# Distributed-Deep-Learning/ps

Measured on AMD Instinct MI355X. Metric: samples/sec (whole node) ResNet-50 sync-BSP at 1/2/4/8 MI355X workers, higher is better.
Workload: dtype bf16; 1 GPU; model=ResNet-50, global_batch=1024, image_size=224, parallelism=ps-bsp-colocated-dp1, optimizer=momentum@lr:0.1@momentum:0.9@wd:5e-05@nesterov:0.0@, staleness=0, fused_bn=True, ranks_per_device=1, compute_priority=high, side_stream=True, streams_per_rank=3, data_plane=local

## Files before the change

### csrc/kernels/conv_bwd_fused.hip

```cpp
#include <algorithm>
#include <cstdlib>

#include "psamd_device.h"
#include "psamd_launch.h"

namespace psamd {
namespace {

typedef float f32x16 __attribute__((ext_vector_type(16)));
typedef short s16x4 __attribute__((ext_vector_type(4)));
typedef short s16x8 __attribute__((ext_vector_type(8)));
typedef short s16x8i __attribute__((ext_vector_type(8)));
typedef __attribute__((address_space(1))) const void gptr_t;
typedef __attribute__((address_space(3))) void lptr_t;
typedef __attribute__((address_space(3))) const char lds_char;

__device__ __attribute__((aligned(16))) uint16_t kZeroRow[8] = {0, 0, 0, 0, 0, 0, 0, 0};

constexpr int kTM = 128;
constexpr int kKS = 64;
constexpr int kNW = 8;
constexpr int kSlot = kTM * kKS * 2;

__device__ __forceinline__ int swf(int r) {
  const int y = (r >> 1) & 7;
  return y ^ ((y & 1) << 2);
}

__device__ __forceinline__ uint32_t lds_addr(const void* p) {
  return static_cast<uint32_t>(reinterpret_cast<uintptr_t>((lds_char*)p));
}

__device__ __forceinline__ bf16x8_t ld_b128(uint32_t a) {
  bf16x8_t v;
  asm volatile("ds_read_b128 %0, %1" : "=v"(v) : "v"(a) : "memory");
  return v;
}
__device__ __forceinline__ f32x4 ld_f4(uint32_t a) {
  f32x4 v;
  asm volatile("ds_read_b128 %0, %1" : "=v"(v) : "v"(a) : "memory");
  return v;
}
__device__ __forceinline__ s16x4 ld_b64(uint32_t a) {
  s16x4 v;
  asm volatile("ds_read_b64 %0, %1" : "=v"(v) : "v"(a) : "memory");
  return v;
}
__device__ __forceinline__ s16x4 ld_tr(uint32_t a) {
  s16x4 v;
  asm volatile("ds_read_b64_tr_b16 %0, %1" : "=v"(v) : "v"(a) : "memory");
  return v;
}
__device__ __forceinline__ void st_b128(uint32_t a, bf16x8_t v) {
  asm volatile("ds_write_b128 %0, %1" ::"v"(a), "v"(v) : "memory");
}
__device__ __forceinline__ void lgkm0() { asm volatile("s_waitcnt lgkmcnt(0)" ::: "memory"); }
template <typename T>
__device__ __forceinline__ void tie(T& v) {
  asm volatile("" : "+v"(v));
}
template <int N>
__device__ __forceinline__ void wait_vm() {
  asm volatile("s_waitcnt vmcnt(%0)" ::"n"(N) : "memory");
}
__device__ __forceinline__ void lds_bar() {
  asm volatile("s_waitcnt lgkmcnt(0)" ::: "memory");
  __builtin_amdgcn_s_barrier();
  asm volatile("" ::: "memory");
}

__device__ __forceinline__ bf16x8_t cat8(s16x4 lo, s16x4 hi) {
  return __builtin_bit_cast(bf16x8_t, s16x8{lo[0], lo[1], lo[2], lo[3], hi[0], hi[1], hi[2], hi[3]});
}

template <int CI, int CO, bool PLAIN>
__global__ __launch_bounds__(512, 1) void conv11_bwd_fused_kernel(const Conv11BwdArgs p) {
  static_assert(CI == 64 && CO == 256, "the layer-1 conv3 shape (64 -> 256): 4 stages per tile");
  constexpr int NS = CO / kKS;
  constexpr int NR = 5, PD = NR - 1;
  constexpr int WROW = CO * 2;
  constexpr int W_BYTES = CI * WROW;
  constexpr int RING = W_BYTES;
  constexpr int Z2 = RING + NR * kSlot;
  constexpr int PAR = Z2 + 2 * kSlot;
  constexpr int NPAR = 3 * CO + 4 * CI;
  constexpr int LDS_BYTES = PAR + NPAR * 4;
  static_assert(LDS_BYTES <= 163840, "LDS budget");
  static_assert(4 * NS * 16 * 64 * 4 <= (NR + 2) * kSlot, "dW half-sum scratch fits the ring + z2 slots");
  __shared__ __attribute__((aligned(16))) uint8_t lds[LDS_BYTES];
  float* const par = reinterpret_cast<float*>(lds + PAR);
  const uint32_t L0 = lds_addr(lds);

  const int t = threadIdx.x, lane = t & 63, wave = __builtin_amdgcn_readfirstlane(t >> 6);
  const int fr = lane & 31, fh = lane >> 5;
  const int GM = gridDim.x, mg = blockIdx.x;
  const int ntiles = (p.M + kTM - 1) / kTM;
  const int my_tiles = mg < ntiles ? (ntiles - mg + GM - 1) / GM : 0;
  const int nq = my_tiles * NS;
  auto stage_m0 = [&](int q) { return q < nq ? (mg + (q / NS) * GM) * kTM : p.M; };

  for (int i = t; i < NPAR; i += kNW * 64) {
    float v;
    if (i < 3 * CO) v = p.cbwd[i];
    else if (PLAIN) v = 0.f;
    else if (i < 3 * CO + 2 * CI) v = p.cf2[i - 3 * CO];
    else if (i < 3 * CO + 3 * CI) v = p.mean2[i - 3 * CO - 2 * CI];
    else v = p.invstd2[i - 3 * CO - 3 * CI];
    par[i] = v;
  }
  {
    constexpr int CPR = CO / 8, RPP = 64 / CPR, PPW = W_BYTES / 1024 / kNW;
    const int lr = lane / CPR, lp = lane % CPR;
#pragma unroll
    for (int i = 0; i < PPW; ++i) {
      const int k = wave * PPW + i, r = k * RPP + lr;
      __builtin_amdgcn_global_load_lds((gptr_t*)(p.wt + static_cast<int64_t>(r) * CO + (lp ^ (r & 15)) * 8),
                                       (lptr_t*)(lds + k * 1024), 16, 0, 0);
    }
  }
  auto issue_tile = [&](const uint16_t* base, int stride, int col0, int m0, int dst) {
#pragma unroll
    for (int i = 0; i < 2; ++i) {
      const int k = wave * 2 + i, r = 8 * k + (lane >> 3), m = m0 + r;
      const int lc = (lane & 7) ^ swf(r);
      const uint16_t* src = m < p.M ? base + static_cast<int64_t>(m) * stride + col0 + lc * 8 : kZeroRow;
      __builtin_amdgcn_global_load_lds((gptr_t*)src, (lptr_t*)(lds + dst + k * 1024), 16, 0, 0);
    }
  };
  const int zr = t >> 3, zc = t & 7;
  u16x8 z3r[2][2];
  auto load_z3 = [&](int q, u16x8 (&dst)[2]) {
    const int m0 = stage_m0(q), col = (q % NS) * kKS + zc * 8;
#pragma unroll
    for (int i = 0; i < 2; ++i) {
      const int m = m0 + zr + 64 * i;
      dst[i] = m < p.M ? *reinterpret_cast<const u16x8*>(p.z3 + static_cast<int64_t>(m) * CO + col)
                       : u16x8{0, 0, 0, 0, 0, 0, 0, 0};
    }
  };
  issue_tile(p.z2, CI, 0, stage_m0(0), Z2);
#pragma unroll
  for (int i = 0; i < PD; ++i) issue_tile(p.g, CO, (i % NS) * kKS, stage_m0(i), RING + i * kSlot);
  load_z3(0, z3r[0]);
  load_z3(1, z3r[1]);
  wait_vm<0>();
  lds_bar();

  const int pb = wave & 3, cbd = wave >> 2;
  const int nb = wave & 1, cw = (wave >> 1) & 1, khw = wave >> 2;
  const int dpx = 32 * pb + fr, dsw = swf(dpx);
  const uint32_t wrow = L0 + static_cast<uint32_t>((32 * cbd + fr) * WROW);
  const int gi = lane >> 4, i16 = lane & 15;
  const int trow = 8 * (gi >> 1) + (i16 >> 2), tcol = 16 * (gi & 1) + 4 * (i16 & 3);
  auto tr_off = [&](int c0, int h) {
    const int r = trow + 4 * h;
    return static_cast<uint32_t>(r * 128 + ((((c0 + tcol) >> 3) ^ swf(r)) << 4) + (tcol & 7) * 2);
  };
  const uint32_t tD0 = tr_off(32 * nb, 0), tD1 = tr_off(32 * nb, 1);
  const uint32_t tZ0 = tr_off(32 * cw, 0), tZ1 = tr_off(32 * cw, 1);
  const float asc = par[3 * CO + 32 * cw + fr], ash = par[3 * CO + CI + 32 * cw + fr];

  f32x16 acc_dg, accW[NS];
  auto zero16 = [](f32x16& a) {
#pragma unroll
    for (int i = 0; i < 16; ++i) a[i] = 0.f;
  };
  zero16(acc_dg);
#pragma unroll
  for (int s = 0; s < NS; ++s) zero16(accW[s]);
  const int ec = 32 * cbd + fr;
  const float emc = par[3 * CO + ec], esh = par[3 * CO + CI + ec], emu = par[3 * CO + 2 * CI + ec],
              eis = par[3 * CO + 3 * CI + ec];
  float s1 = 0.f, s2 = 0.f;

  bf16x8_t a2f[4];
  auto make_a2 = [&](int ti) {
    const uint32_t zs = L0 + Z2 + (ti & 1) * kSlot + khw * (4 * 2048);
    s16x4 lo[4], hi[4];
#pragma unroll
    for (int ks = 0; ks < 4; ++ks) {
      lo[ks] = ld_tr(zs + ks * 2048 + tZ0);
      hi[ks] = ld_tr(zs + ks * 2048 + tZ1);
    }
    lgkm0();
#pragma unroll
    for (int ks = 0; ks < 4; ++ks) {
      tie(lo[ks]);
      tie(hi[ks]);
      if constexpr (PLAIN) {
        a2f[ks] = cat8(lo[ks], hi[ks]);
        continue;
      }
      u16x8 v = __builtin_bit_cast(u16x8, cat8(lo[ks], hi[ks]));
#pragma unroll
      for (int j = 0; j < 8; ++j) v[j] = f32_to_bf16(bf16_to_f32(v[j]) * asc + ash);
      const s16x8i z = {0, 0, 0, 0, 0, 0, 0, 0};
      a2f[ks] = __builtin_bit_cast(bf16x8_t, __builtin_elementwise_max(__builtin_bit_cast(s16x8i, v), z));
    }
  };
  auto transform = [&](int sl, int s, int m0, const u16x8 (&z3v)[2]) {
    const uint32_t ds = L0 + RING + sl * kSlot;
    const uint32_t pa = L0 + PAR + (s * kKS + zc * 8) * 4;
    const f32x4 ca0 = ld_f4(pa), ca1 = ld_f4(pa + 16);
    const f32x4 cb0 = ld_f4(pa + CO * 4), cb1 = ld_f4(pa + CO * 4 + 16);
    const f32x4 cc0 = ld_f4(pa + 2 * CO * 4), cc1 = ld_f4(pa + 2 * CO * 4 + 16);
    bf16x8_t gv[2];
    uint32_t ga[2];
#pragma unroll
    for (int i = 0; i < 2; ++i) {
      const int r = zr + 64 * i;
      ga[i] = ds + r * 128 + ((zc ^ swf(r)) << 4);
      gv[i] = ld_b128(ga[i]);
    }
    lgkm0();
    f32x4 c0a = ca0, c0b = ca1, c1a = cb0, c1b = cb1, c2a = cc0, c2b = cc1;
    tie(c0a); tie(c0b); tie(c1a); tie(c1b); tie(c2a); tie(c2b);
#pragma unroll
    for (int i = 0; i < 2; ++i) {
      tie(gv[i]);
      const u16x8 g8 = __builtin_bit_cast(u16x8, gv[i]);
      const u16x8 z8 = z3v[i];
      u16x8 d;
#pragma unroll
      for (int j = 0; j < 8; ++j) {
        const float a = j < 4 ? c0a[j] : c0b[j - 4], b = j < 4 ? c1a[j] : c1b[j - 4], c = j < 4 ? c2a[j] : c2b[j - 4];
        d[j] = f32_to_bf16(a * bf16_to_f32(g8[j]) + b * bf16_to_f32(z8[j]) + c);
      }
      if (m0 + zr + 64 * i >= p.M) d = u16x8{0, 0, 0, 0, 0, 0, 0, 0};
      st_b128(ga[i], __builtin_bit_cast(bf16x8_t, d));
    }
  };
  auto compute = [&](int sl, f32x16& aw, int s) {
    const uint32_t ds = L0 + RING + sl * kSlot;
#pragma unroll
    for (int h = 0; h < 2; ++h) {
      bf16x8_t wa[2], xb[2];
      s16x4 dlo[2], dhi[2];
#pragma unroll
      for (int k2 = 0; k2 < 2; ++k2) {
        const int ks = 2 * h + k2;
        wa[k2] = ld_b128(wrow + ((((8 * s + 2 * ks + fh) ^ (fr & 15))) << 4));
        xb[k2] = ld_b128(ds + dpx * 128 + (((2 * ks + fh) ^ dsw) << 4));
        dlo[k2] = ld_tr(ds + (4 * khw + ks) * 2048 + tD0);
        dhi[k2] = ld_tr(ds + (4 * khw + ks) * 2048 + tD1);
      }
      lgkm0();
#pragma unroll
      for (int k2 = 0; k2 < 2; ++k2) {
        tie(wa[k2]);
        tie(xb[k2]);
        tie(dlo[k2]);
        tie(dhi[k2]);
      }
#pragma unroll
      for (int k2 = 0; k2 < 2; ++k2)
        acc_dg = __builtin_amdgcn_mfma_f32_32x32x16_bf16(xb[k2], wa[k2], acc_dg, 0, 0, 0);
#pragma unroll
      for (int k2 = 0; k2 < 2; ++k2)
        aw = __builtin_amdgcn_mfma_f32_32x32x16_bf16(cat8(dlo[k2], dhi[k2]), a2f[2 * h + k2], aw, 0, 0, 0);
    }
  };
  auto epilogue = [&](int ti) {
    const int m0 = (mg + ti * GM) * kTM;
    if constexpr (PLAIN) {
#pragma unroll
      for (int q = 0; q < 16; ++q) {
        const int m = m0 + 32 * pb + 8 * (q >> 2) + 4 * fh + (q & 3);
        if (m < p.M) p.gy[static_cast<int64_t>(m) * CI + ec] = f32_to_bf16(acc_dg[q]);
      }
      zero16(acc_dg);
      return;
    }
    const uint32_t zs = L0 + Z2 + (ti & 1) * kSlot;
    s16x4 zv[4];
#pragma unroll
    for (int q4 = 0; q4 < 4; ++q4) {
      const int r = 32 * pb + 8 * q4 + 4 * (gi >> 1) + (i16 >> 2);
      const int col = 32 * cbd + 16 * (gi & 1) + 4 * (i16 & 3);
      zv[q4] = ld_tr(zs + r * 128 + (((col >> 3) ^ swf(r)) << 4) + (col & 7) * 2);
    }
    lgkm0();
#pragma unroll
    for (int q4 = 0; q4 < 4; ++q4) {
      tie(zv[q4]);
      const u16x4 z4 = __builtin_bit_cast(u16x4, zv[q4]);
#pragma unroll
      for (int e = 0; e < 4; ++e) {
        const uint16_t val = f32_to_bf16(acc_dg[4 * q4 + e]);
        const float z = bf16_to_f32(z4[e]);
        const bool on = z * emc + esh > 0.f;
        const float gv = on ? bf16_to_f32(val) : 0.f;
        s1 += gv;
        s2 += gv * ((z - emu) * eis);
        const int m = m0 + 32 * pb + 8 * q4 + 4 * fh + e;
        if (m < p.M) p.gy[static_cast<int64_t>(m) * CI + ec] = on ? val : static_cast<uint16_t>(0);
      }
    }
    zero16(acc_dg);
  };

  int sl = 0, q = 0;
  for (int ti = 0; ti < my_tiles; ++ti) {
    const int m0 = (mg + ti * GM) * kTM;
#pragma unroll
    for (int s = 0; s < NS; ++s, ++q) {
      if (s == 0) make_a2(ti);
      transform(sl, s, m0, z3r[s & 1]);
      lds_bar();
      const int slp = sl == 0 ? NR - 1 : sl - 1;
      issue_tile(p.g, CO, ((q + PD) % NS) * kKS, stage_m0(q + PD), RING + slp * kSlot);
      load_z3(q + 2, z3r[s & 1]);
      if (s == 0) issue_tile(p.z2, CI, 0, ti + 1 < my_tiles ? m0 + GM * kTM : p.M, Z2 + ((ti + 1) & 1) * kSlot);
      compute(sl, accW[s], s);
      if (s == NS - 1) epilogue(ti);
      if (s == NS - 1) wait_vm<6>();
      else wait_vm<8>();
      lds_bar();
      sl = sl == NR - 1 ? 0 : sl + 1;
    }
  }
  wait_vm<0>();
  lds_bar();

  s1 += __shfl_xor(s1, 32, 64);
  s2 += __shfl_xor(s2, 32, 64);
  float* red = reinterpret_cast<float*>(lds + RING);
  if (!PLAIN && fh == 0) {
    red[pb * CI + ec] = s1;
    red[(4 + pb) * CI + ec] = s2;
  }
  __syncthreads();
  if (!PLAIN && t < CI) {
    p.part[static_cast<int64_t>(mg) * CI + t] = (red[t] + red[CI + t]) + (red[2 * CI + t] + red[3 * CI + t]);
    p.part[static_cast<int64_t>(GM + mg) * CI + t] =
        (red[4 * CI + t] + red[5 * CI + t]) + (red[6 * CI + t] + red[7 * CI + t]);
  }
  __syncthreads();
  float* wsc = reinterpret_cast<float*>(lds + RING);
  if (khw == 1) {
#pragma unroll
    for (int s = 0; s < NS; ++s)
#pragma unroll
      for (int i = 0; i < 16; ++i) wsc[(((wave - 4) * NS + s) * 16 + i) * 64 + lane] = accW[s][i];
  }
  __syncthreads();
  if (khw == 0) {
    float* slab = p.ws + static_cast<int64_t>(mg) * CO * CI;
#pragma unroll
    for (int s = 0; s < NS; ++s)
#pragma unroll
      for (int i = 0; i < 16; ++i) {
        const int n = s * kKS + 32 * nb + 8 * (i >> 2) + 4 * fh + (i & 3);
        slab[n * CI + 32 * cw + fr] = accW[s][i] + wsc[((wave * NS + s) * 16 + i) * 64 + lane];
      }
  }
}

template <bool BF16>
__global__ __launch_bounds__(256) void slab_sum_kernel(const float* __restrict__ in, int nslab, int per, int64_t E,
                                                       void* __restrict__ out) {
  const int64_t e = static_cast<int64_t>(blockIdx.x) * 256 + threadIdx.x;
  if (e >= E) return;
  const int b0 = blockIdx.y * per, b1 = min(nslab, b0 + per);
  float a0 = 0.f, a1 = 0.f, a2 = 0.f, a3 = 0.f;
  int b = b0;
  for (; b + 3 < b1; b += 4) {
    a0 += in[b * E + e];
    a1 += in[(b + 1) * E + e];
    a2 += in[(b + 2) * E + e];
    a3 += in[(b + 3) * E + e];
  }
  for (; b < b1; ++b) a0 += in[b * E + e];
  const float v = (a0 + a1) + (a2 + a3);
  if constexpr (BF16) static_cast<uint16_t*>(out)[blockIdx.y * E + e] = f32_to_bf16(v);
  else static_cast<float*>(out)[blockIdx.y * E + e] = v;
}

int slab_levels(int nslab) { return nslab > 16 ? (nslab + 15) / 16 : 0; }

}

bool conv11_bwd_fused_ok(int CI, int CO) { return CI == 64 && CO == 256; }

bool conv11_bwd_plain_ok(int CI, int CO) { return CI == 64 && CO == 256; }

bool conv11_bwd_built(int CI, int CO) { return CI == 64 && CO == 256; }

int conv11_bwd_blocks(int M, int CI, int CO) {
  (void)CI, (void)CO;
  const int ntiles = (M + kTM - 1) / kTM;
  return std::max(1, std::min(ntiles, 256));
}

int64_t conv11_bwd_ws(int M, int CI, int CO) {
  const int gm = conv11_bwd_blocks(M, CI, CO);
  return static_cast<int64_t>(gm + slab_levels(gm)) * CI * CO;
}

void launch_conv11_bwd_fused(const Conv11BwdArgs& a, int CI, int CO, hipStream_t s) {
  if (a.M <= 0) return;
  const int gm = conv11_bwd_blocks(a.M, CI, CO);
  if (CI == 64 && CO == 256 && a.cf2 == nullptr)
    hipLaunchKernelGGL((conv11_bwd_fused_kernel<64, 256, true>), dim3(gm), dim3(512), 0, s, a);
  else if (CI == 64 && CO == 256) hipLaunchKernelGGL((conv11_bwd_fused_kernel<64, 256, false>), dim3(gm), dim3(512), 0, s, a);
  else if (a.cf2 == nullptr) return;
  else return;
  const int64_t E = static_cast<int64_t>(CI) * CO;
  const unsigned eb = static_cast<unsigned>((E + 255) / 256);
  const int groups = slab_levels(gm);
  if (groups) {
    float* mid = a.ws + static_cast<int64_t>(gm) * E;
    hipLaunchKernelGGL(slab_sum_kernel<false>, dim3(eb, groups), dim3(256), 0, s, a.ws, gm, 16, E,
                       static_cast<void*>(mid));
    hipLaunchKernelGGL(slab_sum_kernel<true>, dim3(eb), dim3(256), 0, s, mid, groups, groups, E,
                       static_cast<void*>(a.dw));
  } else {
    hipLaunchKernelGGL(slab_sum_kernel<true>, dim3(eb), dim3(256), 0, s, a.ws, gm, gm, E, static_cast<void*>(a.dw));
  }
}

}
```

### csrc/kernels/convgemm.hip

```cpp
#include <algorithm>
#include <cstdlib>
#include <type_traits>

#include "psamd_device.h"
#include "psamd_launch.h"

namespace psamd {
namespace {

typedef float f32x16 __attribute__((ext_vector_type(16)));
typedef short s16x4 __attribute__((ext_vector_type(4)));
typedef short s16x8 __attribute__((ext_vector_type(8)));
typedef __attribute__((address_space(3))) s16x4 lds_s16x4;

constexpr int kBM = 128;
constexpr int kBK = 64;
constexpr int kWM = 64;

__device__ __forceinline__ bf16x8_t as_bf16x8(s16x8 v) { return __builtin_bit_cast(bf16x8_t, v); }

__device__ __forceinline__ void lds_barrier() {
  asm volatile("s_waitcnt lgkmcnt(0)" ::: "memory");
  __builtin_amdgcn_s_barrier();
  asm volatile("" ::: "memory");
// ... 1202 lines not shown
  for (int st = 0; st < pre; ++st) issue(st, st);
  if constexpr (PROL) {
    if (pre == 3) wait_vmcnt<2 * PER>();
    else if (pre == 2) wait_vmcnt<PER>();
    else wait_vmcnt<0>();
    lds_barrier();
    if (nst > 0) xform(0);
  }
  for (int st = 0; st < nst; ++st) {
    const int ahead = min(WS - 2, nst - 1 - st);
    if constexpr (PROL) {
      if (ahead >= 2) wait_vmcnt<PER>();
      else wait_vmcnt<0>();
    } else {
      if (ahead >= 2) wait_vmcnt<2 * PER>();
      else if (ahead == 1) wait_vmcnt<PER>();
      else wait_vmcnt<0>();
    }
    lds_barrier();
    if (st + WS - 1 < nst) issue(st + WS - 1, (st + WS - 1) % WS);
    if constexpr (PROL) {
      if (st + 1 < nst) xform((st + 1) % WS);
    }
    if constexpr (DB) {
      if (dbt) {
        const uint16_t* Gs = lds + (st % WS) * STAGE;
        const int cc = t % GCPR;
#pragma unroll
        for (int r = t / GCPR; r < kWP; r += DBR) {
          const u16x8 v = *reinterpret_cast<const u16x8*>(Gs + r * BNO + ((cc ^ tr_swz<BNO>(r)) << 3));
#pragma unroll
          for (int j = 0; j < 8; ++j) dbacc[j] += bf16_to_f32(v[j]);
        }
      }
    }
    mma(st % WS);
  }
  if constexpr (DB) {
    if (dbt) {
      lds_barrier();
      float* red = reinterpret_cast<float*>(lds);
#pragma unroll
      for (int j = 0; j < 8; ++j) red[t * 8 + j] = dbacc[j];
      lds_barrier();
      if (t < BNO) {
        const int cc = t >> 3, j = t & 7;
        float sum = 0.f;
        for (int k = 0; k < DBR; ++k) sum += red[(k * GCPR + cc) * 8 + j];
        p.dbws[static_cast<int64_t>(split) * p.N + n0 + t] = sum;
      }
    }
  }
  float* sl = p.ws + static_cast<int64_t>(split) * p.N * p.K;
  const int h = lane >> 5, kl = lane & 31;
#pragma unroll
  for (int i = 0; i < TN; ++i)
#pragma unroll
    for (int j = 0; j < TK; ++j)
#pragma unroll
      for (int q = 0; q < 16; ++q) {
        const int n = n0 + wn + 32 * i + (q & 3) + 8 * (q >> 2) + 4 * h;
        sl[static_cast<int64_t>(n) * p.K + k0 + wk + 32 * j + kl] = acc[i][j][q];
      }
}

constexpr int kPP = 112;

template <int OFF>
__device__ __forceinline__ s16x4 ds_tr_off(uint32_t a) {
  s16x4 v;
  asm volatile("ds_read_b64_tr_b16 %0, %1 offset:%2" : "=v"(v) : "v"(a), "i"(OFF) : "memory");
  return v;
}

template <int W, int S>
__global__ __launch_bounds__(768, 1) void conv_wgrad_patch_kernel(const ConvWgradArgs p, int stages_per_split) {
  constexpr int OW = W / S, R = kPP / OW, PR = S * (R - 1) + 3;
  constexpr int PW = S == 1 ? W + 2 : (W + 2) / 2;
  constexpr int KPS = S == 1 ? 3 : 2;
  static_assert(kPP % OW == 0 && OW % 4 == 0 && W % S == 0, "a stage is whole rows; 4-pixel groups stay in a row");
  constexpr int GPL = kPP * 64;
  constexpr int GB = 2 * GPL;
  constexpr int PPL = S * PR * PW * 64;
  constexpr int PB = ((2 * PPL + 1023) / 1024) * 1024;
  constexpr int GI = GB / 1024, PI = PB / 1024;
  constexpr int NI = GI + PI;
  constexpr int STB = GB + PB;
  constexpr int MAXW = (NI + 11) / 12;
  static_assert(GB % 1024 == 0 && MAXW <= 8 && (KPS == 2 || MAXW <= 4) && KPS * STB <= 160 * 1024, "stage shape");
  __shared__ __attribute__((aligned(16))) uint16_t lds[KPS * STB / 2];

  const ConvGeo& g = p.g;
  const int t = threadIdx.x, lane = t & 63, wave = __builtin_amdgcn_readfirstlane(t >> 6);
  const int nct = g.C / 64, tiles = (p.N / 64) * nct;
  const int L = xcd_remap(blockIdx.x, gridDim.x);
  const int split = L / tiles, tile = L - split * tiles;
  const int n0 = (tile / nct) * 64, c0 = (tile % nct) * 64;
  const int rows_per_img = g.OH / R, total = p.M / kPP;
  const int sb = split * stages_per_split;
  const int se = min(total, sb + stages_per_split);
  const int nst = se > sb ? se - sb : 0;

  const int myn = (NI - wave + 11) / 12;
  auto issue = [&](int st, int buf) {
    const int q = sb + st, img = q / rows_per_img, ih0 = (q - img * rows_per_img) * R * S - 1;
    uint8_t* base = reinterpret_cast<uint8_t*>(lds) + buf * STB;
    const uint16_t* gsrc = p.dz + static_cast<int64_t>(q) * kPP * p.N + n0;
    const uint16_t* xsrc = p.x + (static_cast<int64_t>(img) * g.H + ih0) * g.W * g.C + c0;
#pragma unroll
    for (int j = 0; j < MAXW; ++j) {
      if (j >= myn) break;
      const int i = wave + 12 * j;
      const uint16_t* src;
      if (i < GI) {
        const int ch = i * 64 + lane, pl = ch / (GPL / 16), r = ch - pl * (GPL / 16);
        src = gsrc + static_cast<int64_t>(r >> 2) * p.N + pl * 32 + (r & 3) * 8;
      } else {
        const int ch = (i - GI) * 64 + lane, pl = ch / (PPL / 16), r = ch - pl * (PPL / 16), slot = r >> 2;
        const int par = slot / (PR * PW), rem = slot - par * (PR * PW), pr = rem / PW;
        const int pc = S * (rem - pr * PW) + par, ih = ih0 + pr;
        const bool ok = pl < 2 && pc >= 1 && pc <= W && static_cast<unsigned>(ih) < static_cast<unsigned>(g.H);
        src = ok ? xsrc + (static_cast<int64_t>(pr) * W + (pc - 1)) * g.C + pl * 32 + (r & 3) * 8 : kZeroPage;
      }
      __builtin_amdgcn_global_load_lds((gptr_t*)src, (lptr_t*)(base + i * 1024), 16, 0, 0);
    }
  };

  const int kh = wave % 3, nh = (wave / 3) & 1, chf = wave / 6;
  const int gi = lane >> 4, i16 = lane & 15;
  const int mrow = 8 * (gi >> 1) + (i16 >> 2), colb = (16 * (gi & 1) + 4 * (i16 & 3)) * 2;
  const uint32_t ga = static_cast<uint32_t>(nh * GPL + mrow * 64 + colb);
  uint32_t xa[7][2];
#pragma unroll
  for (int s = 0; s < 7; ++s)
#pragma unroll
    for (int h = 0; h < 2; ++h) {
      const int m = 16 * s + 4 * h + mrow, oh = m / OW, ow = m - oh * OW;
      xa[s][h] = static_cast<uint32_t>(GB + chf * PPL + ((S * oh + kh) * PW + ow) * 64 + colb);
    }

  f32x16 acc[3];
#pragma unroll
  for (int k = 0; k < 3; ++k)
#pragma unroll
    for (int q = 0; q < 16; ++q) acc[k][q] = 0.f;
  auto mma = [&](int buf) {
    const uint32_t b0 = static_cast<uint32_t>(reinterpret_cast<uintptr_t>((const lds_s16x4*)lds)) + buf * STB;
    const uint32_t gb = b0 + ga;
    constexpr int K1 = S == 1 ? 64 : PR * PW * 64, K2 = S == 1 ? 128 : 64;
#define PSAMD_PATCH_STEP(Q)                                                                              \
  {                                                                                                      \
    s16x4 a0 = ds_tr_off<(16 * Q) * 64>(gb), a1 = ds_tr_off<(16 * Q + 4) * 64>(gb);                      \
    const uint32_t x0 = b0 + xa[Q][0], x1 = b0 + xa[Q][1];                                               \
    s16x4 p00 = ds_tr_off<0>(x0), p01 = ds_tr_off<0>(x1);                                                \
    s16x4 p10 = ds_tr_off<K1>(x0), p11 = ds_tr_off<K1>(x1);                                              \
    s16x4 p20 = ds_tr_off<K2>(x0), p21 = ds_tr_off<K2>(x1);                                              \
       \
       \
    asm volatile("s_waitcnt lgkmcnt(0)"                                                                  \
                 : "+v"(a0), "+v"(a1), "+v"(p00), "+v"(p01), "+v"(p10), "+v"(p11), "+v"(p20), "+v"(p21)  \
                 :                                                                                       \
                 : "memory");                                                                            \
    const bf16x8_t af = as_bf16x8(s16x8{a0[0], a0[1], a0[2], a0[3], a1[0], a1[1], a1[2], a1[3]});        \
    acc[0] = __builtin_amdgcn_mfma_f32_32x32x16_bf16(                                                    \
        af, as_bf16x8(s16x8{p00[0], p00[1], p00[2], p00[3], p01[0], p01[1], p01[2], p01[3]}), acc[0], 0, 0, 0); \
    acc[1] = __builtin_amdgcn_mfma_f32_32x32x16_bf16(                                                    \
        af, as_bf16x8(s16x8{p10[0], p10[1], p10[2], p10[3], p11[0], p11[1], p11[2], p11[3]}), acc[1], 0, 0, 0); \
    acc[2] = __builtin_amdgcn_mfma_f32_32x32x16_bf16(                                                    \
        af, as_bf16x8(s16x8{p20[0], p20[1], p20[2], p20[3], p21[0], p21[1], p21[2], p21[3]}), acc[2], 0, 0, 0); \
  }
    PSAMD_PATCH_STEP(0)
    PSAMD_PATCH_STEP(1)
    PSAMD_PATCH_STEP(2)
    PSAMD_PATCH_STEP(3)
    PSAMD_PATCH_STEP(4)
    PSAMD_PATCH_STEP(5)
    PSAMD_PATCH_STEP(6)
#undef PSAMD_PATCH_STEP
  };

  const int pre = nst < KPS - 1 ? nst : KPS - 1;
  for (int st = 0; st < pre; ++st) issue(st, st);
  for (int st = 0; st < nst; ++st) {
    if (KPS == 3 && st + 1 < nst) {
      if (myn == 4) asm volatile("s_waitcnt vmcnt(4)" ::: "memory");
      else if (myn == 3) asm volatile("s_waitcnt vmcnt(3)" ::: "memory");
      else if (myn == 2) asm volatile("s_waitcnt vmcnt(2)" ::: "memory");
      else asm volatile("s_waitcnt vmcnt(0)" ::: "memory");
    } else {
      asm volatile("s_waitcnt vmcnt(0)" ::: "memory");
    }
    lds_barrier();
    if (st + KPS - 1 < nst) issue(st + KPS - 1, (st + KPS - 1) % KPS);
    mma(st % KPS);
  }
  float* sl = p.ws + static_cast<int64_t>(split) * p.N * p.K;
  const int h = lane >> 5, cl = lane & 31;
#pragma unroll
  for (int kw = 0; kw < 3; ++kw)
#pragma unroll
    for (int q = 0; q < 16; ++q) {
      const int n = n0 + nh * 32 + (q & 3) + 8 * (q >> 2) + 4 * h;
      const int k = (kh * 3 + kw) * g.C + c0 + chf * 32 + cl;
      sl[static_cast<int64_t>(n) * p.K + k] = acc[kw][q];
    }
// ... 439 lines not shown
```

### ps_amd/knobs.py

```python
from __future__ import annotations

import os
from typing import Dict, FrozenSet

ENV = "PS_AMD_DISABLE"

ROUTES: Dict[str, str] = {
    "fused_block": "bottlenecks module by module (nn.Conv2d on MIOpen + BatchNormAct2d)",
    "conv3x3": "fused blocks' 3x3 convolutions on MIOpen instead of the implicit-GEMM kernels",
    "block_out": "block outputs applied by their own pass, not in the next conv1's prologue",
    "fold_bn3": "bn3's backward reduce as its own pass, not in the consumer's conv1 data-gradient epilogue",
    "fold_bn_ds": "the downsample BN's backward reduce as its own pass (epilogue 8 instead of 9)",
    "conv3_bwd_fused": "conv3's data + weight gradient as two GEMMs (dz3 through HBM)",
    "ds_bwd_fused": "the downsample's data + weight gradient as apply pass + two GEMMs",
    "weight_prep": "backward weight layouts built per block instead of in one launch per forward",
    "pool_bn_bwd": "stem max-pool backward and BN backward as separate passes",
    "stem_bwd_fused": "stem weight gradient reading a materialised dz",
    "splitk_wgrad": "linear weight gradients on hipBLASLt instead of the split-K kernel",
    "linear_fork": "linear weight gradients on the compute stream",
    "fused_relu": "Linear + ReLU as separate ops",
    "ps_linear": "PS-owned linear weight gradients through autograd's ordinary accumulation",
    "fused_attn": "short-sequence attention on SDPA",
    "flash_attn": "causal GQA attention on SDPA",
    "fused_xent": "cross-entropy on fp32 logits through F.cross_entropy",
    "bag_pool": "multi-hot bags pooled by gather_rows -> weight multiply -> segment_reduce_rows ([nnz, dim] in HBM)",
}

_cache: Dict[str, FrozenSet[str]] = {}


def _parse(raw: str) -> FrozenSet[str]:
    got = _cache.get(raw)
    if got is None:
        got = frozenset(s.strip() for s in raw.split(",") if s.strip())
        bad = sorted(got - set(ROUTES))
        if bad:
            raise ValueError(f"{ENV}: unknown route(s) {bad}; known: {sorted(ROUTES)}")
        _cache[raw] = got
    return got


def disabled(route: str) -> bool:
    if route not in ROUTES:
        raise KeyError(f"unknown route {route!r}")
    raw = os.environ.get(ENV)
    return bool(raw) and route in _parse(raw)


def enabled(route: str) -> bool:
    return not disabled(route)
```

### ps_amd/ops/convgemm.py

```python
from __future__ import annotations

import contextlib
import enum
import threading
import weakref
from typing import List

import torch
import torch.nn as nn
import torch.nn.functional as F

from .. import knobs
from . import side_stream as _side
from ._ext import native


def rows(x: torch.Tensor) -> torch.Tensor:
    n, c, h, w = x.shape
    if not x.is_contiguous(memory_format=torch.channels_last):
        x = x.contiguous(memory_format=torch.channels_last)
    return x.permute(0, 2, 3, 1).reshape(n * h * w, c)


def image(y2: torch.Tensor, n: int, h: int, w: int) -> torch.Tensor:
# ... 64 lines not shown
                parts.append((((ar2 * 3 + kh) * 3 + kw) * c1 + ar1).reshape(-1))
        idx = _PHASE_IDX[key] = torch.cat(parts).to(w.device)
    flat = w.permute(0, 2, 3, 1).reshape(-1)[idx]
    out, o = [], 0
    for nh, nw in ((1, 1), (1, 2), (2, 1), (2, 2)):
        k = nh * nw * c2
        out.append(flat[o:o + c1 * k].view(c1, k))
        o += c1 * k
    return out


DGRAD_S2_MIN_C = 128

WGRAD3X3_MIN_C = 256

TWOSRC_MAX_N = 128

PRO_FUSE_MAX_K = 256


def _conv3x3_enabled() -> bool:
    return knobs.enabled("conv3x3")


class _Link:

    __slots__ = ("out_ref", "z3", "bits", "mean", "invstd", "part", "dx_ptr", "dx_version", "dx_keep", "zd", "md",
                 "idd")

    def __init__(self, z3, bits, mean, invstd, zd=None, md=None, idd=None):
        self.out_ref = None
        self.z3, self.bits, self.mean, self.invstd = z3, bits, mean, invstd
        self.zd, self.md, self.idd = zd, md, idd
        self.part = None
        self.dx_ptr = self.dx_version = self.dx_keep = None


FOLD_STATS = {"used": 0, "ds": 0, "resp": 0}


class _Deferred:

    __slots__ = ("out_ref", "z3", "cf3", "res", "cfd", "out", "bits")

    def __init__(self, z3, cf3, res, cfd, out, bits):
        self.out_ref = None
        self.z3, self.cf3, self.res, self.cfd, self.out, self.bits = z3, cf3, res, cfd, out, bits

    def flush(self) -> None:
        y, b = native().bn_apply_coef(self.z3, self.cf3, self.res, self.cfd, 1, True)
        with torch.no_grad():
            self.out.copy_(y)
            self.bits.copy_(b)


def _resp_enabled() -> bool:
    return knobs.enabled("block_out")


def big_tile(m: int, n: int, k: int, src2: int = Src2.NONE, epi: int = Epi.STATS, pro: bool = False) -> bool:
    return tuple(native().conv_gemm_plan(m, n, k, [m, 1, m, 1, 1, 1, 0], pro, int(epi), int(src2))[:2]) == (256, 256)


def resp_consumer_ok(blk: nn.Module, m: int = 0) -> bool:
    c1 = blk.conv1
    if m > 0 and big_tile(m, c1.out_channels, c1.in_channels, src2=Src2.BLOCK_OUT):
        return True
    return c1.out_channels <= TWOSRC_MAX_N and (
        c1.in_channels >= 64 * native().kTwosrcGldsMinNk or c1.out_channels <= 64)


def flush_deferred() -> None:
    pend = getattr(_tls, "pend", None)
    _tls.pend = None
    if pend is not None and pend.out_ref is not None and pend.out_ref() is not None:
        pend.flush()


def _bwd_prologue_enabled(n: int) -> bool:
    return n <= TWOSRC_MAX_N


def _conv3_bwd_fused(ci: int, co: int) -> bool:
    return knobs.enabled("conv3_bwd_fused") and bool(native().conv11_bwd_fused_supported(ci, co))


def _ds_bwd_fused(ci: int, co: int, s: int) -> bool:
    return (s == 1 and knobs.enabled("ds_bwd_fused")
            and bool(native().conv11_bwd_fused_supported(ci, co, True)))


def _fold_enabled() -> bool:
    return knobs.enabled("fold_bn3")


def _fold_ds_enabled() -> bool:
    return knobs.enabled("fold_bn_ds")


def _conv1_dgrad_epi(downsample: bool, stride: int, fold: bool, producer_ds: bool) -> Epi:
    if downsample:
        if stride == 2:
            return Epi.FOLD_ADD_S2 if fold else Epi.ADD_S2
        return Epi.FOLD_ADD if fold else Epi.ADD
    if not fold:
        return Epi.ADD_MASKED
    return Epi.FOLD_ADD_MASKED_DS if producer_ds else Epi.FOLD_ADD_MASKED


class _BottleneckFn(torch.autograd.Function):
    @staticmethod
    def forward(ctx, x, w1, g1, b1, w2, g2, b2, w3, g3, b3, wd, gd, bd, blk, link_in, pend_in):
        nat = native()
        n, cin, h, w = x.shape
        s = blk.conv2.stride[0]
        oh, ow = (h - 1) // s + 1, (w - 1) // s + 1
        gi, go = geo(h, w), geo(oh, ow)
        x2 = rows(x)
        bn1, bn2, bn3 = blk.bn1, blk.bn2, blk.bn3
        k1 = bn1.running_mean
        if pend_in is not None:
            z1, p1 = nat.conv_gemm(pend_in.z3, _mat(w1), gi, pro=pend_in.cf3, epi=Epi.STATS, kshift=k1,
                                   a2=pend_in.res, pro2=pend_in.cfd, aout=x2, abits=pend_in.bits)
            FOLD_STATS["resp"] += 1
        else:
            z1, p1 = nat.conv_gemm(x2, _mat(w1), gi, epi=Epi.STATS, kshift=k1)
        m1, i1, cf1 = _finalize(p1, k1, n * h * w, bn1)
        y1 = nat.bn_apply_coef(z1, cf1, None, None, 1)[0]
        if _conv3x3_enabled():
            k2 = bn2.running_mean
            z2r, p2s = nat.conv_gemm(y1, _mat3(w2), geo(h, w, 3, s, 1), epi=Epi.STATS, kshift=k2)
            m2, i2, cf2 = _finalize(p2s, k2, n * oh * ow, bn2)
        else:
            z2r = rows(F.conv2d(image(y1, n, h, w), w2, None, s, 1))
            m2, i2, cf2 = nat.bn_stats(z2r, g2, b2, bn2.running_mean, bn2.running_var, True, _momentum(bn2),
                                       float(bn2.eps))
        k3 = bn3.running_mean
        if z2r.shape[1] <= PRO_FUSE_MAX_K:
            z3, p3 = nat.conv_gemm(z2r, _mat(w3), go, pro=cf2, epi=Epi.STATS, kshift=k3)
        else:
            z3, p3 = nat.conv_gemm(nat.bn_apply_coef(z2r, cf2, None, None, 1)[0], _mat(w3), go, epi=Epi.STATS,
                                   kshift=k3)
        m3, i3, cf3 = _finalize(p3, k3, n * oh * ow, bn3)
        cfd = None
        if wd is not None:
            bnd = blk.downsample[1]
            kd = bnd.running_mean
            zd, pd = nat.conv_gemm(x2, _mat(wd), geo(h, w, 1, s), epi=Epi.STATS, kshift=kd)
            md, idd, cfd = _finalize(pd, kd, n * oh * ow, bnd)
        else:
            zd = md = idd = None
        if (getattr(blk, "_defer_out", False) and getattr(_tls, "pending", None) is not None
                and _resp_enabled()):
            out = torch.empty_like(z3)
            obits = torch.empty(z3.numel() // 8, dtype=torch.uint8, device=z3.device)
            _tls.pend_new = _Deferred(z3, cf3, zd if wd is not None else x2, cfd, out, obits)
        else:
            out, obits = nat.bn_apply_coef(z3, cf3, zd if wd is not None else x2, cfd, 1, True)
        ctx.save_for_backward(x2, w1, w2, w3, wd, g1, g2, g3, gd, z1, y1, z2r, z3, obits, zd,
                              m1, i1, cf1, m2, i2, cf2, m3, i3, md, idd)
        ctx.dims = (n, h, w, s, oh, ow)
        ctx.prep = _prep_for(blk, w1, w2, w3)
        ctx.link_in = link_in
        ctx.link_out = (_Link(z3, obits, m3, i3, zd if _fold_ds_enabled() else None, md, idd)
                        if _fold_enabled() else None)
        return image(out, n, oh, ow)
# ... 263 lines not shown
```

Before: 16910 samples/s.

## Extend fused conv3 backward kernel to layer-2 128->512 shape via channel halves

Generalizes the fused 1x1 conv3 data+weight-gradient backward kernel to the layer-2 shape (128 in, 512 out). It splits the input channels into two 64-wide halves handled by paired blocks and uses a 3-slot ring to fit LDS. Per-lane constants are re-read from LDS to relieve register pressure. This replaces two separate GEMMs with dz3 going through HBM for layer 2. A side change in the strided conv GEMM shrinks the parameter staging buffer so a small block can be co-resident; this risks lower pipelining depth and extra LDS reads.

Result: no change. 17020 samples/s (median of 6 runs) (+0.7%).

```diff
diff --git a/csrc/kernels/conv_bwd_fused.hip b/csrc/kernels/conv_bwd_fused.hip
--- a/csrc/kernels/conv_bwd_fused.hip
+++ b/csrc/kernels/conv_bwd_fused.hip
@@ -41,6 +41,11 @@
   asm volatile("ds_read_b128 %0, %1" : "=v"(v) : "v"(a) : "memory");
   return v;
 }
+__device__ __forceinline__ float ld_f1(uint32_t a) {
+  float v;
+  asm volatile("ds_read_b32 %0, %1" : "=v"(v) : "v"(a) : "memory");
+  return v;
+}
 __device__ __forceinline__ s16x4 ld_b64(uint32_t a) {
   s16x4 v;
   asm volatile("ds_read_b64 %0, %1" : "=v"(v) : "v"(a) : "memory");
@@ -73,11 +78,14 @@
   return __builtin_bit_cast(bf16x8_t, s16x8{lo[0], lo[1], lo[2], lo[3], hi[0], hi[1], hi[2], hi[3]});
 }
 
-template <int CI, int CO, bool PLAIN>
+template <int CIF, int CO, bool PLAIN>
 __global__ __launch_bounds__(512, 1) void conv11_bwd_fused_kernel(const Conv11BwdArgs p) {
-  static_assert(CI == 64 && CO == 256, "the layer-1 conv3 shape (64 -> 256): 4 stages per tile");
+  static_assert((CIF == 64 && CO == 256) || (CIF == 128 && CO == 512 && !PLAIN),
+                "the layer-1 (64 -> 256) and layer-2 (128 -> 512, two channel halves) conv3 shapes");
+  constexpr int CI = 64;
+  constexpr int HALVES = CIF / CI;
   constexpr int NS = CO / kKS;
-  constexpr int NR = 5, PD = NR - 1;
+  constexpr int NR = CO == 256 ? 5 : 3, PD = NR - 1;
   constexpr int WROW = CO * 2;
   constexpr int W_BYTES = CI * WROW;
   constexpr int RING = W_BYTES;
@@ -86,14 +94,28 @@
   constexpr int NPAR = 3 * CO + 4 * CI;
   constexpr int LDS_BYTES = PAR + NPAR * 4;
   static_assert(LDS_BYTES <= 163840, "LDS budget");
-  static_assert(4 * NS * 16 * 64 * 4 <= (NR + 2) * kSlot, "dW half-sum scratch fits the ring + z2 slots");
+  constexpr int WSC_BYTES = 4 * NS * 16 * 64 * 4;
+  constexpr int WSC = WSC_BYTES <= (NR + 2) * kSlot ? RING : 0;
+  static_assert(WSC + WSC_BYTES <= PAR, "dW half-sum scratch fits below the parameters");
   __shared__ __attribute__((aligned(16))) uint8_t lds[LDS_BYTES];
   float* const par = reinterpret_cast<float*>(lds + PAR);
   const uint32_t L0 = lds_addr(lds);
 
   const int t = threadIdx.x, lane = t & 63, wave = __builtin_amdgcn_readfirstlane(t >> 6);
   const int fr = lane & 31, fh = lane >> 5;
-  const int GM = gridDim.x, mg = blockIdx.x;
+  int GM = gridDim.x, mg = blockIdx.x, half = 0;
+  if constexpr (HALVES == 2) {
+    const int bid = blockIdx.x;
+    GM = gridDim.x >> 1;
+    if ((GM & 7) == 0) {
+      half = (bid >> 3) & 1;
+      mg = (bid >> 4) * 8 + (bid & 7);
+    } else {
+      half = bid & 1;
+      mg = bid >> 1;
+    }
+  }
+  const int hc = half * CI;
   const int ntiles = (p.M + kTM - 1) / kTM;
   const int my_tiles = mg < ntiles ? (ntiles - mg + GM - 1) / GM : 0;
   const int nq = my_tiles * NS;
@@ -103,9 +125,10 @@
     float v;
     if (i < 3 * CO) v = p.cbwd[i];
     else if (PLAIN) v = 0.f;
-    else if (i < 3 * CO + 2 * CI) v = p.cf2[i - 3 * CO];
-    else if (i < 3 * CO + 3 * CI) v = p.mean2[i - 3 * CO - 2 * CI];
-    else v = p.invstd2[i - 3 * CO - 3 * CI];
+    else if (i < 3 * CO + CI) v = p.cf2[hc + i - 3 * CO];
+    else if (i < 3 * CO + 2 * CI) v = p.cf2[CIF + hc + i - 3 * CO - CI];
+    else if (i < 3 * CO + 3 * CI) v = p.mean2[hc + i - 3 * CO - 2 * CI];
+    else v = p.invstd2[hc + i - 3 * CO - 3 * CI];
     par[i] = v;
   }
   {
@@ -114,7 +137,7 @@
 #pragma unroll
     for (int i = 0; i < PPW; ++i) {
       const int k = wave * PPW + i, r = k * RPP + lr;
-      __builtin_amdgcn_global_load_lds((gptr_t*)(p.wt + static_cast<int64_t>(r) * CO + (lp ^ (r & 15)) * 8),
+      __builtin_amdgcn_global_load_lds((gptr_t*)(p.wt + static_cast<int64_t>(hc + r) * CO + (lp ^ (r & 15)) * 8),
                                        (lptr_t*)(lds + k * 1024), 16, 0, 0);
     }
   }
@@ -138,7 +161,7 @@
                        : u16x8{0, 0, 0, 0, 0, 0, 0, 0};
     }
   };
-  issue_tile(p.z2, CI, 0, stage_m0(0), Z2);
+  issue_tile(p.z2, CIF, hc, stage_m0(0), Z2);
 #pragma unroll
   for (int i = 0; i < PD; ++i) issue_tile(p.g, CO, (i % NS) * kKS, stage_m0(i), RING + i * kSlot);
   load_z3(0, z3r[0]);
@@ -160,6 +183,10 @@
   const uint32_t tZ0 = tr_off(32 * cw, 0), tZ1 = tr_off(32 * cw, 1);
   const float asc = par[3 * CO + 32 * cw + fr], ash = par[3 * CO + CI + 32 * cw + fr];
 
+  auto fresh = [](auto v) {
+    if constexpr (NS > 4) tie(v);
+    return v;
+  };
   f32x16 acc_dg, accW[NS];
   auto zero16 = [](f32x16& a) {
 #pragma unroll
@@ -176,13 +203,24 @@
   bf16x8_t a2f[4];
   auto make_a2 = [&](int ti) {
     const uint32_t zs = L0 + Z2 + (ti & 1) * kSlot + khw * (4 * 2048);
+    const uint32_t z0 = fresh(tZ0), z1 = fresh(tZ1);
+    float sc = asc, sh = ash;
+    if constexpr (NS > 4) {
+      const uint32_t pa = L0 + PAR + (3 * CO + 32 * cw + fresh(fr)) * 4;
+      sc = ld_f1(pa);
+      sh = ld_f1(pa + CI * 4);
+    }
     s16x4 lo[4], hi[4];
 #pragma unroll
     for (int ks = 0; ks < 4; ++ks) {
-      lo[ks] = ld_tr(zs + ks * 2048 + tZ0);
-      hi[ks] = ld_tr(zs + ks * 2048 + tZ1);
+      lo[ks] = ld_tr(zs + ks * 2048 + z0);
+      hi[ks] = ld_tr(zs + ks * 2048 + z1);
     }
     lgkm0();
+    if constexpr (NS > 4) {
+      tie(sc);
+      tie(sh);
+    }
 #pragma unroll
     for (int ks = 0; ks < 4; ++ks) {
       tie(lo[ks]);
@@ -193,14 +231,14 @@
       }
       u16x8 v = __builtin_bit_cast(u16x8, cat8(lo[ks], hi[ks]));
 #pragma unroll
-      for (int j = 0; j < 8; ++j) v[j] = f32_to_bf16(bf16_to_f32(v[j]) * asc + ash);
+      for (int j = 0; j < 8; ++j) v[j] = f32_to_bf16(bf16_to_f32(v[j]) * sc + sh);
       const s16x8i z = {0, 0, 0, 0, 0, 0, 0, 0};
       a2f[ks] = __builtin_bit_cast(bf16x8_t, __builtin_elementwise_max(__builtin_bit_cast(s16x8i, v), z));
     }
   };
   auto transform = [&](int sl, int s, int m0, const u16x8 (&z3v)[2]) {
     const uint32_t ds = L0 + RING + sl * kSlot;
-    const uint32_t pa = L0 + PAR + (s * kKS + zc * 8) * 4;
+    const uint32_t pa = L0 + PAR + (s * kKS + fresh(zc) * 8) * 4;
     const f32x4 ca0 = ld_f4(pa), ca1 = ld_f4(pa + 16);
     const f32x4 cb0 = ld_f4(pa + CO * 4), cb1 = ld_f4(pa + CO * 4 + 16);
     const f32x4 cc0 = ld_f4(pa + 2 * CO * 4), cc1 = ld_f4(pa + 2 * CO * 4 + 16);
@@ -232,6 +270,8 @@
   };
   auto compute = [&](int sl, f32x16& aw, int s) {
     const uint32_t ds = L0 + RING + sl * kSlot;
+    const uint32_t wr = fresh(wrow), d0 = fresh(tD0), d1 = fresh(tD1);
+    const int fx = fresh(fr & 15), px = fresh(dpx), sx = fresh(dsw);
 #pragma unroll
     for (int h = 0; h < 2; ++h) {
       bf16x8_t wa[2], xb[2];
@@ -239,10 +279,10 @@
 #pragma unroll
       for (int k2 = 0; k2 < 2; ++k2) {
         const int ks = 2 * h + k2;
-        wa[k2] = ld_b128(wrow + ((((8 * s + 2 * ks + fh) ^ (fr & 15))) << 4));
-        xb[k2] = ld_b128(ds + dpx * 128 + (((2 * ks + fh) ^ dsw) << 4));
-        dlo[k2] = ld_tr(ds + (4 * khw + ks) * 2048 + tD0);
-        dhi[k2] = ld_tr(ds + (4 * khw + ks) * 2048 + tD1);
+        wa[k2] = ld_b128(wr + ((((8 * s + 2 * ks + fh) ^ fx)) << 4));
+        xb[k2] = ld_b128(ds + px * 128 + (((2 * ks + fh) ^ sx) << 4));
+        dlo[k2] = ld_tr(ds + (4 * khw + ks) * 2048 + d0);
+        dhi[k2] = ld_tr(ds + (4 * khw + ks) * 2048 + d1);
       }
       lgkm0();
 #pragma unroll
@@ -266,20 +306,35 @@
 #pragma unroll
       for (int q = 0; q < 16; ++q) {
         const int m = m0 + 32 * pb + 8 * (q >> 2) + 4 * fh + (q & 3);
-        if (m < p.M) p.gy[static_cast<int64_t>(m) * CI + ec] = f32_to_bf16(acc_dg[q]);
+        if (m < p.M) p.gy[static_cast<int64_t>(m) * CIF + hc + ec] = f32_to_bf16(acc_dg[q]);
       }
       zero16(acc_dg);
       return;
     }
     const uint32_t zs = L0 + Z2 + (ti & 1) * kSlot;
+    const int il = fresh(i16);
+    float mc = emc, msh = esh, mu = emu, is = eis;
+    if constexpr (NS > 4) {
+      const uint32_t pa = L0 + PAR + (3 * CO + fresh(ec)) * 4;
+      mc = ld_f1(pa);
+      msh = ld_f1(pa + CI * 4);
+      mu = ld_f1(pa + 2 * CI * 4);
+      is = ld_f1(pa + 3 * CI * 4);
+    }
     s16x4 zv[4];
 #pragma unroll
     for (int q4 = 0; q4 < 4; ++q4) {
-      const int r = 32 * pb + 8 * q4 + 4 * (gi >> 1) + (i16 >> 2);
-      const int col = 32 * cbd + 16 * (gi & 1) + 4 * (i16 & 3);
+      const int r = 32 * pb + 8 * q4 + 4 * (gi >> 1) + (il >> 2);
+      const int col = 32 * cbd + 16 * (gi & 1) + 4 * (il & 3);
       zv[q4] = ld_tr(zs + r * 128 + (((col >> 3) ^ swf(r)) << 4) + (col & 7) * 2);
     }
     lgkm0();
+    if constexpr (NS > 4) {
+      tie(mc);
+      tie(msh);
+      tie(mu);
+      tie(is);
+    }
 #pragma unroll
     for (int q4 = 0; q4 < 4; ++q4) {
       tie(zv[q4]);
@@ -288,12 +343,12 @@
       for (int e = 0; e < 4; ++e) {
         const uint16_t val = f32_to_bf16(acc_dg[4 * q4 + e]);
         const float z = bf16_to_f32(z4[e]);
-        const bool on = z * emc + esh > 0.f;
+        const bool on = z * mc + msh > 0.f;
         const float gv = on ? bf16_to_f32(val) : 0.f;
         s1 += gv;
-        s2 += gv * ((z - emu) * eis);
+        s2 += gv * ((z - mu) * is);
         const int m = m0 + 32 * pb + 8 * q4 + 4 * fh + e;
-        if (m < p.M) p.gy[static_cast<int64_t>(m) * CI + ec] = on ? val : static_cast<uint16_t>(0);
+        if (m < p.M) p.gy[static_cast<int64_t>(m) * CIF + hc + ec] = on ? val : static_cast<uint16_t>(0);
       }
     }
     zero16(acc_dg);
@@ -310,11 +365,17 @@
       const int slp = sl == 0 ? NR - 1 : sl - 1;
       issue_tile(p.g, CO, ((q + PD) % NS) * kKS, stage_m0(q + PD), RING + slp * kSlot);
       load_z3(q + 2, z3r[s & 1]);
-      if (s == 0) issue_tile(p.z2, CI, 0, ti + 1 < my_tiles ? m0 + GM * kTM : p.M, Z2 + ((ti + 1) & 1) * kSlot);
+      if (s == 0) issue_tile(p.z2, CIF, hc, ti + 1 < my_tiles ? m0 + GM * kTM : p.M, Z2 + ((ti + 1) & 1) * kSlot);
       compute(sl, accW[s], s);
       if (s == NS - 1) epilogue(ti);
-      if (s == NS - 1) wait_vm<6>();
-      else wait_vm<8>();
+      if constexpr (NR == 5) {
+        if (s == NS - 1) wait_vm<6>();
+        else wait_vm<8>();
+      } else {
+        static_assert(NR == 3 && NS > 2, "counted waits of the 3-slot ring");
+        if (s < PD) wait_vm<6>();
+        else wait_vm<4>();
+      }
       lds_bar();
       sl = sl == NR - 1 ? 0 : sl + 1;
     }
@@ -331,12 +392,16 @@
   }
   __syncthreads();
   if (!PLAIN && t < CI) {
-    p.part[static_cast<int64_t>(mg) * CI + t] = (red[t] + red[CI + t]) + (red[2 * CI + t] + red[3 * CI + t]);
-    p.part[static_cast<int64_t>(GM + mg) * CI + t] =
-        (red[4 * CI + t] + red[5 * CI + t]) + (red[6 * CI + t] + red[7 * CI + t]);
+    const int64_t r0 = static_cast<int64_t>(blockIdx.x) * CIF, r1 = static_cast<int64_t>(gridDim.x + blockIdx.x) * CIF;
+    p.part[r0 + hc + t] = (red[t] + red[CI + t]) + (red[2 * CI + t] + red[3 * CI + t]);
+    p.part[r1 + hc + t] = (red[4 * CI + t] + red[5 * CI + t]) + (red[6 * CI + t] + red[7 * CI + t]);
+    if constexpr (HALVES == 2) {
+      p.part[r0 + (CI - hc) + t] = 0.f;
+      p.part[r1 + (CI - hc) + t] = 0.f;
+    }
   }
   __syncthreads();
-  float* wsc = reinterpret_cast<float*>(lds + RING);
+  float* wsc = reinterpret_cast<float*>(lds + WSC);
   if (khw == 1) {
 #pragma unroll
     for (int s = 0; s < NS; ++s)
@@ -345,13 +410,13 @@
   }
   __syncthreads();
   if (khw == 0) {
-    float* slab = p.ws + static_cast<int64_t>(mg) * CO * CI;
+    float* slab = p.ws + static_cast<int64_t>(mg) * CO * CIF + hc;
 #pragma unroll
     for (int s = 0; s < NS; ++s)
 #pragma unroll
       for (int i = 0; i < 16; ++i) {
         const int n = s * kKS + 32 * nb + 8 * (i >> 2) + 4 * fh + (i & 3);
-        slab[n * CI + 32 * cw + fr] = accW[s][i] + wsc[((wave * NS + s) * 16 + i) * 64 + lane];
+        slab[n * CIF + 32 * cw + fr] = accW[s][i] + wsc[((wave * NS + s) * 16 + i) * 64 + lane];
       }
   }
 }
@@ -380,30 +445,35 @@
 
 }
 
-bool conv11_bwd_fused_ok(int CI, int CO) { return CI == 64 && CO == 256; }
+bool conv11_bwd_fused_ok(int CI, int CO) { return (CI == 64 && CO == 256) || (CI == 128 && CO == 512); }
 
 bool conv11_bwd_plain_ok(int CI, int CO) { return CI == 64 && CO == 256; }
 
-bool conv11_bwd_built(int CI, int CO) { return CI == 64 && CO == 256; }
+bool conv11_bwd_built(int CI, int CO) { return (CI == 64 && CO == 256) || (CI == 128 && CO == 512); }
+
+namespace {
+int conv11_bwd_halves(int CI) { return CI == 128 ? 2 : 1; }
+}
 
 int conv11_bwd_blocks(int M, int CI, int CO) {
-  (void)CI, (void)CO;
-  const int ntiles = (M + kTM - 1) / kTM;
-  return std::max(1, std::min(ntiles, 256));
+  (void)CO;
+  const int ntiles = (M + kTM - 1) / kTM, hv = conv11_bwd_halves(CI);
+  return hv * std::max(1, std::min(ntiles, 256 / hv));
 }
 
 int64_t conv11_bwd_ws(int M, int CI, int CO) {
-  const int gm = conv11_bwd_blocks(M, CI, CO);
+  const int gm = conv11_bwd_blocks(M, CI, CO) / conv11_bwd_halves(CI);
   return static_cast<int64_t>(gm + slab_levels(gm)) * CI * CO;
 }
 
 void launch_conv11_bwd_fused(const Conv11BwdArgs& a, int CI, int CO, hipStream_t s) {
   if (a.M <= 0) return;
-  const int gm = conv11_bwd_blocks(a.M, CI, CO);
+  const int nblk = conv11_bwd_blocks(a.M, CI, CO), gm = nblk / conv11_bwd_halves(CI);
   if (CI == 64 && CO == 256 && a.cf2 == nullptr)
-    hipLaunchKernelGGL((conv11_bwd_fused_kernel<64, 256, true>), dim3(gm), dim3(512), 0, s, a);
-  else if (CI == 64 && CO == 256) hipLaunchKernelGGL((conv11_bwd_fused_kernel<64, 256, false>), dim3(gm), dim3(512), 0, s, a);
+    hipLaunchKernelGGL((conv11_bwd_fused_kernel<64, 256, true>), dim3(nblk), dim3(512), 0, s, a);
+  else if (CI == 64 && CO == 256) hipLaunchKernelGGL((conv11_bwd_fused_kernel<64, 256, false>), dim3(nblk), dim3(512), 0, s, a);
   else if (a.cf2 == nullptr) return;
+  else if (CI == 128 && CO == 512) hipLaunchKernelGGL((conv11_bwd_fused_kernel<128, 512, false>), dim3(nblk), dim3(512), 0, s, a);
   else return;
   const int64_t E = static_cast<int64_t>(CI) * CO;
   const unsigned eb = static_cast<unsigned>((E + 255) / 256);
diff --git a/csrc/kernels/convgemm.hip b/csrc/kernels/convgemm.hip
--- a/csrc/kernels/convgemm.hip
+++ b/csrc/kernels/convgemm.hip
@@ -1308,12 +1308,14 @@
   constexpr int GPL = kPP * 64;
   constexpr int GB = 2 * GPL;
   constexpr int PPL = S * PR * PW * 64;
-  constexpr int PB = ((2 * PPL + 1023) / 1024) * 1024;
-  constexpr int GI = GB / 1024, PI = PB / 1024;
+  constexpr int PB = S == 1 ? ((2 * PPL + 1023) / 1024) * 1024 : 2 * PPL;
+  constexpr int GI = GB / 1024, PI = (PB + 1023) / 1024;
   constexpr int NI = GI + PI;
   constexpr int STB = GB + PB;
   constexpr int MAXW = (NI + 11) / 12;
   static_assert(GB % 1024 == 0 && MAXW <= 8 && (KPS == 2 || MAXW <= 4) && KPS * STB <= 160 * 1024, "stage shape");
+  static_assert(PB % 16 == 0 && (S == 1 ? PB % 1024 == 0 : KPS * STB + 1536 <= 160 * 1024),
+                "whole DMA pieces, or LDS left for a co-resident 1 KiB block");
   __shared__ __attribute__((aligned(16))) uint16_t lds[KPS * STB / 2];
 
   const ConvGeo& g = p.g;
@@ -1347,6 +1349,7 @@
         const int pc = S * (rem - pr * PW) + par, ih = ih0 + pr;
         const bool ok = pl < 2 && pc >= 1 && pc <= W && static_cast<unsigned>(ih) < static_cast<unsigned>(g.H);
         src = ok ? xsrc + (static_cast<int64_t>(pr) * W + (pc - 1)) * g.C + pl * 32 + (r & 3) * 8 : kZeroPage;
+        if (PB % 1024 != 0 && ch >= PB / 16) continue;
       }
       __builtin_amdgcn_global_load_lds((gptr_t*)src, (lptr_t*)(base + i * 1024), 16, 0, 0);
     }
diff --git a/ps_amd/knobs.py b/ps_amd/knobs.py
--- a/ps_amd/knobs.py
+++ b/ps_amd/knobs.py
@@ -12,6 +12,7 @@
     "fold_bn3": "bn3's backward reduce as its own pass, not in the consumer's conv1 data-gradient epilogue",
     "fold_bn_ds": "the downsample BN's backward reduce as its own pass (epilogue 8 instead of 9)",
     "conv3_bwd_fused": "conv3's data + weight gradient as two GEMMs (dz3 through HBM)",
+    "conv3_bwd_fused_l2": "the same two GEMMs for the 128 -> 512 (layer-2) conv3 only",
     "ds_bwd_fused": "the downsample's data + weight gradient as apply pass + two GEMMs",
     "weight_prep": "backward weight layouts built per block instead of in one launch per forward",
     "pool_bn_bwd": "stem max-pool backward and BN backward as separate passes",
diff --git a/ps_amd/ops/convgemm.py b/ps_amd/ops/convgemm.py
--- a/ps_amd/ops/convgemm.py
+++ b/ps_amd/ops/convgemm.py
@@ -170,6 +170,8 @@
 
 
 def _conv3_bwd_fused(ci: int, co: int) -> bool:
+    if ci == 128 and knobs.disabled("conv3_bwd_fused_l2"):
+        return False
     return knobs.enabled("conv3_bwd_fused") and bool(native().conv11_bwd_fused_supported(ci, co))
 
 
```
